# delta-mpc/delta-node

Measured on AMD Instinct MI355X. Metric: elements/s device-resident Shamir 3-of-5 split+recombine, 2^24 vec, 1/2/4/8 GPU, higher is better.
Workload: dtype u32

## Files before the change

delta-node_amd/csrc/dn_internal.hpp:

```cpp
#pragma once

#include <cstddef>
#include <cstdint>
#include <cstdlib>

#include "dn_shamir.h"

struct ihipEvent_t;
struct ihipStream_t;

namespace dn {
inline const char* tune_env(const char* name) {
#ifdef DN_TUNING
  return std::getenv(name);
#else
  (void)name;
  return nullptr;
#endif
}

int set_error(int code, const char* fmt, ...) __attribute__((format(printf, 2, 3)));

inline bool fd_needs_fold(int t, int n) {
  double s = 0.0, p = 1.0;
  for (int j = 0; j < t; ++j) {
    s += p;
    p *= static_cast<double>(n + t);
  }
  return s >= 8388608.0;
}

int device_cu_count();

struct StageBuf {
  void* p = nullptr;
  size_t bytes = 0;
  ::ihipEvent_t* ev = nullptr;
  int dev = -1;
};
StageBuf stage_take(size_t need);
void stage_give(StageBuf b, ::ihipStream_t* const* s);

uint64_t mt_jump_words();
uint64_t mt_jump_max_subs();
void mt_advance_window(const uint32_t* win, uint64_t steps, uint32_t* out);
bool mt_final_state(const uint32_t* state, int idx, uint64_t words, uint32_t* fin, int32_t* fidx);

constexpr uint64_t kMtRtRows = 2048;
const uint64_t* mt_direct_rows_l14(uint64_t S, uint64_t* version);
bool mt_rt_rows_compute(uint64_t* out, uint64_t nrows);
bool mt_xpow_mod(uint64_t e, uint64_t* out);
void mt_rt_rows_checksum(const uint64_t* words, uint64_t n, uint64_t out[2]);
}
```

delta-node_amd/csrc/host_gf2poly.cpp:

```cpp
#include <immintrin.h>

#include <cstdint>
#include <cstring>
#include <mutex>
#include <vector>

#include "dn_internal.hpp"

namespace dn {
namespace {

#include "mt19937_charpoly.inc"
#include "mt19937_jump.inc"
#include "mt19937_jump_direct.inc"

constexpr int kW = kMtPolyWords;
constexpr int kDeg = 19937;
static_assert(kW * 64 > kDeg && (kW - 1) * 64 <= kDeg, "poly words");

const uint64_t kP[1][kW] = DN_MT_CHAR_POLY;
const uint64_t kJump14[kMtJumpRows][kW] = DN_MT_JUMP_POLYS;
const uint64_t kDirect14[kMtDirectRows][kW] = DN_MT_JUMP_DIRECT_L14;

__attribute__((target("pclmul,sse4.1"))) void clmul_poly(const uint64_t* a, int na, const uint64_t* b, int nb,
                                                          uint64_t* r) {
  std::memset(r, 0, sizeof(uint64_t) * (na + nb));
  for (int k = 0; k < na + nb - 1; ++k) {
    const int i0 = k - nb + 1 > 0 ? k - nb + 1 : 0, i1 = k < na - 1 ? k : na - 1;
    __m128i acc = _mm_setzero_si128(), acc2 = _mm_setzero_si128();
    int i = i0;
    for (; i + 1 <= i1; i += 2) {
      const __m128i av = _mm_loadu_si128(reinterpret_cast<const __m128i*>(a + i));
      const __m128i bv = _mm_loadu_si128(reinterpret_cast<const __m128i*>(b + k - i - 1));
      acc = _mm_xor_si128(acc, _mm_clmulepi64_si128(av, bv, 0x10));
      acc2 = _mm_xor_si128(acc2, _mm_clmulepi64_si128(av, bv, 0x01));
    }
    if (i <= i1)
      acc = _mm_xor_si128(acc, _mm_clmulepi64_si128(_mm_loadl_epi64(reinterpret_cast<const __m128i*>(a + i)),
                                                     _mm_loadl_epi64(reinterpret_cast<const __m128i*>(b + k - i)), 0x00));
    acc = _mm_xor_si128(acc, acc2);
    r[k] ^= static_cast<uint64_t>(_mm_cvtsi128_si64(acc));
    r[k + 1] ^= static_cast<uint64_t>(_mm_extract_epi64(acc, 1));
  }
}

void shr_bits(const uint64_t* a, int na, int sh, uint64_t* out, int n) {
  const int ws = sh / 64, bs = sh % 64;
  for (int i = 0; i < n; ++i) {
    const int k = i + ws;
    const uint64_t lo = k < na ? a[k] : 0u;
    const uint64_t hi = k + 1 < na ? a[k + 1] : 0u;
    out[i] = bs ? (lo >> bs) | (hi << (64 - bs)) : lo;
  }
}

bool bit(const uint64_t* a, int i) { return (a[i / 64] >> (i % 64)) & 1u; }

// ... 64 lines not shown
    uint64_t h[2];
    mt_rt_rows_checksum(b, nw, h);
    if (h[0] != b[nw] || h[1] != b[nw + 1]) return nullptr;
    for (int s = 1; s <= kMtDirectRows; ++s)
      if (std::memcmp(b + (s - 1) * kW, kDirect14[s - 1], sizeof(uint64_t) * kW)) return nullptr;
    Barrett br;
    std::vector<uint64_t> r(kW);
    for (uint64_t s = kMtRtRows; s > kMtRtRows - 16 * 127; s -= 127) {
      br.mulmod(b + (s - 2) * kW, kJump14[kMtRowB + 1], r.data());
      if (std::memcmp(r.data(), b + (s - 1) * kW, sizeof(uint64_t) * kW)) return nullptr;
    }
    return b;
  }();
  return checked;
}

}

void mt_rt_rows_checksum(const uint64_t* w, uint64_t n, uint64_t out[2]) {
  uint64_t a = 0x9E3779B97F4A7C15ull ^ n, c = 0xC2B2AE3D27D4EB4Full;
  for (uint64_t i = 0; i < n; ++i) {
    a = ((a ^ w[i]) * 0xFF51AFD7ED558CCDull);
    a ^= a >> 29;
    c = ((c + w[i]) * 0xC4CEB9FE1A85EC53ull) ^ (c >> 31) ^ i;
  }
  out[0] = a;
  out[1] = c;
}

bool mt_xpow_mod(uint64_t e, uint64_t* out) {
  if (!__builtin_cpu_supports("pclmul")) return false;
  static Barrett* br = new Barrett;
  std::vector<uint64_t> r(kW, 0), t(kW);
  r[0] = 1;
  for (int b = e ? 63 - __builtin_clzll(e) : -1; b >= 0; --b) {
    br->mulmod(r.data(), r.data(), t.data());
    r.swap(t);
    if ((e >> b) & 1u) {
      uint64_t carry = 0;
      for (int k = 0; k < kW; ++k) {
        const uint64_t w = r[k];
        r[k] = (w << 1) | carry;
        carry = w >> 63;
      }
      if (bit(r.data(), kDeg)) {
        for (int k = 0; k < kW; ++k) r[k] ^= kP[0][k];
      }
    }
  }
  std::memcpy(out, r.data(), sizeof(uint64_t) * kW);
  return true;
}

bool mt_rt_rows_compute(uint64_t* out, uint64_t nrows) {
  if (!__builtin_cpu_supports("pclmul") || nrows == 0) return false;
  Barrett br;
  std::memcpy(out, kDirect14[0], sizeof(uint64_t) * kW);
  for (uint64_t s = 2; s <= nrows; ++s) {
    br.mulmod(out + (s - 2) * kW, kJump14[kMtRowB + 1], out + (s - 1) * kW);
    if (s <= static_cast<uint64_t>(kMtDirectRows) &&
        std::memcmp(out + (s - 1) * kW, kDirect14[s - 1], sizeof(uint64_t) * kW))
      return false;
  }
  return true;
}

const uint64_t* mt_direct_rows_l14(uint64_t S, uint64_t* version) {
  if (S < 2 || S - 1 > kMtRtRows) return nullptr;
  if (const uint64_t* e = embedded_rows()) {
    if (version) *version = ~0ull;
    return e;
  }
  if (!__builtin_cpu_supports("pclmul")) return nullptr;
  Rows& R = rows14();
  std::lock_guard<std::mutex> g(R.m);
  if (!R.ok) return nullptr;
  if (R.rows.empty()) {
    R.rows.assign(static_cast<size_t>(kMtRtRows) * kW, 0u);
    R.have.assign(kMtRtRows, 0u);
    R.br = new Barrett;
    std::memcpy(R.rows.data(), kDirect14[0], sizeof(uint64_t) * kW);
    R.have[0] = 1;
    R.odd_top = 1;
    if (!set_row(R, 2, R.rows.data(), kJump14[kMtRowB + 1])) return nullptr;
  }
  const uint64_t last = S - 1;
  for (uint64_t s = R.odd_top + 2; s <= last; s += 2, R.odd_top += 2)
    if (!set_row(R, s, R.rows.data() + (s - 3) * kW, kJump14[kMtRowB + 2])) return nullptr;
  if (!R.have[last - 1] && !set_row(R, last, R.rows.data() + (last - 2) * kW, kJump14[kMtRowB + 1]))
    return nullptr;
  if (version) *version = R.version;
  return R.rows.data();
}

}

extern "C" int dn_mt19937_rt_rows_embedded(void) { return dn::embedded_rows() ? 1 : 0; }
```

delta-node_amd/csrc/host_mt_jump.cpp:

```cpp
#include <cstdint>
#include <cstring>
#include <vector>

#include "dn_internal.hpp"

namespace dn {
namespace {

#include "mt19937_jump.inc"

alignas(64) static const uint64_t kMtJumpPolys[kMtJumpRows][kMtPolyWords] = DN_MT_JUMP_POLYS;

constexpr int kMtN = 624, kMtM = 397;
constexpr uint32_t kMtA = 0x9908b0dfu, kMtUp = 0x80000000u, kMtLo = 0x7fffffffu;

inline uint32_t mt_mix(uint32_t a, uint32_t b, uint32_t m) {
  const uint32_t y = (a & kMtUp) | (b & kMtLo);
  return m ^ (y >> 1) ^ ((0u - (y & 1u)) & kMtA);
}

__attribute__((target_clones("avx512f", "avx2", "default")))
void mt_extend(uint32_t* __restrict buf, uint64_t p, int steps) {
  const uint32_t* src = buf + p;
  uint32_t* dst = buf + p + kMtN;
// ... 70 lines not shown

uint64_t mt_jump_words() { return kMtJumpL; }
uint64_t mt_jump_max_subs() { return 1ull + static_cast<uint64_t>(kMtJumpRadix) * kMtJumpRadix * kMtJumpRadix; }

bool mt_final_state(const uint32_t* state, int idx, uint64_t words, uint32_t* fin, int32_t* fidx) {
  const uint64_t h = static_cast<uint64_t>(kMtN - idx);
  if (words <= h) {
    std::memcpy(fin, state, kMtN * sizeof(uint32_t));
    *fidx = idx + static_cast<int32_t>(words);
    return true;
  }
  const uint64_t m_end = words - h, q = (m_end + kMtN - 1) / kMtN, tf = kMtN * q;
  const uint64_t sig = (tf + kMtN - 1 - static_cast<uint64_t>(idx)) / kMtJumpL;
  if (sig >= mt_jump_max_subs()) return false;
  std::vector<uint32_t> w(kMtN);
  uint64_t t_sig = 0;
  if (sig == 0) {
    std::memcpy(w.data(), state, kMtN * sizeof(uint32_t));
  } else {
    mt_window_at(state, idx, sig, w.data());
    t_sig = static_cast<uint64_t>(idx) + sig * kMtJumpL - kMtN;
  }
  mt_advance(w.data(), tf - t_sig, fin);
  *fidx = static_cast<int32_t>(m_end - kMtN * (q - 1));
  return true;
}

void mt_advance_window(const uint32_t* win, uint64_t steps, uint32_t* out) { mt_advance(win, steps, out); }

}

using namespace dn;

extern "C" int dn_mt19937_skip(uint32_t* mt_state, int32_t* mt_index, uint64_t words) {
  if (!mt_state || !mt_index) return set_error(DN_ERR_ARG, "dn_mt19937_skip: null pointer");
  const int32_t idx = *mt_index;
  if (idx < 0 || idx > kMtN) return set_error(DN_ERR_ARG, "dn_mt19937_skip: bad MT index");
  std::vector<uint32_t> fin(kMtN);
  int32_t fidx = 0;
  if (!mt_final_state(mt_state, idx, words, fin.data(), &fidx))
    return set_error(DN_ERR_UNSUPPORTED, "dn_mt19937_skip: %llu words exceed the jump table",
                     static_cast<unsigned long long>(words));
  std::memcpy(mt_state, fin.data(), kMtN * sizeof(uint32_t));
  *mt_index = fidx;
  return DN_OK;
}

extern "C" int dn_mt19937_jump_poly(uint64_t words, uint64_t* out) {
  if (!out) return dn::set_error(DN_ERR_ARG, "dn_mt19937_jump_poly: null pointer");
  if (!dn::mt_xpow_mod(words, out))
    return dn::set_error(DN_ERR_UNSUPPORTED, "dn_mt19937_jump_poly: no carry-less multiply");
  return DN_OK;
}
```

delta-node_amd/csrc/mt19937_device.hip:

```cpp
#include <hip/hip_runtime.h>

#include <algorithm>
#include <cstdint>
#include <cstdlib>
#include <cstring>
#include <mutex>
#include <utility>
#include <vector>

#include "dn_internal.hpp"
#include "m521_device.hpp"
#include "mt_plan.hpp"
#include "seg_plan.hpp"

namespace dn {
namespace {

__device__ const uint64_t kMtPolysDev[kMtTabLens][kMtJumpRows][kMtPolyWords] = {
    DN_MT_JUMP_POLYS_L10, DN_MT_JUMP_POLYS_L12, DN_MT_JUMP_POLYS};
__device__ const uint64_t kMtDirectDev[kMtLens][kMtDirectRows][kMtPolyWords] = {
    DN_MT_JUMP_DIRECT_L10, DN_MT_JUMP_DIRECT_L12, DN_MT_JUMP_DIRECT_L14, DN_MT_JUMP_DIRECT_L8};

typedef uint32_t u32x2_t __attribute__((ext_vector_type(2)));
typedef uint32_t u32x4_t __attribute__((ext_vector_type(4)));
// ... 1198 lines not shown
}

struct MtKnobs {
  bool spec = true;
  bool tail_fin = true;
  bool spec_beside = true;
  int beside_cb = 2;
  uint64_t spec_min = 1ull << 23, beside_min = 1ull << 16;
  bool own_by_jumpc = false;
  uint32_t jump_probe = 0;
  bool jump4b = false;
  uint32_t gen_probe = 0;
  bool pc = true;
  uint32_t gen_subs = 0;
  bool force_retry = false;
};

MtKnobs mt_knobs() {
  MtKnobs k;
  auto on = [](const char* n, bool dflt) { const char* e = tune_env(n); return e ? e[0] != '0' : dflt; };
  auto is1 = [](const char* n) { const char* e = tune_env(n); return e && e[0] == '1'; };
  auto num = [](const char* n) { const char* e = tune_env(n); return e ? std::atoi(e) : 0; };
  k.spec = on("DN_MT_SPEC", k.spec);
  k.tail_fin = on("DN_MT_TAIL_FIN", k.tail_fin);
  k.spec_beside = on("DN_MT_SPEC_BESIDE", k.spec_beside);
  if (const char* e = tune_env("DN_MT_BESIDE_CB")) k.beside_cb = e[0] == '2' ? 2 : 3;
  if (const char* e = tune_env("DN_MT_SPEC_MIN")) k.spec_min = std::strtoull(e, nullptr, 10);
  if (const char* e = tune_env("DN_MT_BESIDE_MIN")) k.beside_min = std::strtoull(e, nullptr, 10);
  k.own_by_jumpc = num("DN_MT_SPEC_PROBE") == 5;
  k.jump_probe = static_cast<uint32_t>(num("DN_MT_JUMP_PROBE"));
  k.jump4b = is1("DN_MT_JUMP4B");
  k.gen_probe = static_cast<uint32_t>(num("DN_MT_PROBE"));
  k.pc = on("DN_MT_PC_FORCE", k.pc);
  if (tune_env("DN_MT_GEN_SUBS")) k.gen_subs = static_cast<uint32_t>(std::max(1, num("DN_MT_GEN_SUBS")));
  k.force_retry = is1("DN_MT_FORCE_RETRY");
  return k;
}

struct SpecState {
  std::mutex m;
  hipStream_t side = nullptr, side2 = nullptr;
  hipEvent_t win = nullptr, done = nullptr;
  hipEvent_t j0ev = nullptr, done2 = nullptr;
  bool widx2 = false;
  void* buf[2] = {nullptr, nullptr};
  uint64_t bytes = 0;
  bool armed = false;
  int next = 0;
  uint64_t ncoef = 0;
  int32_t idx = -1;
  uint32_t state[kMtN];
  bool have_end = false;
  uint64_t hits = 0, misses = 0, launched = 0;
  uint64_t* xpow = nullptr;
  uint64_t xpow_words = 0;
  bool xpow_failed = false;
};

std::mutex& spec_table_mutex() {
  static std::mutex* m = new std::mutex;
  return *m;
}
SpecState* spec_slot(int dev) {
  static SpecState* table[16] = {};
  if (dev < 0 || dev >= 16) return nullptr;
  std::lock_guard<std::mutex> g(spec_table_mutex());
  if (!table[dev]) {
    auto* x = new SpecState;
    if (hipStreamCreateWithFlags(&x->side, hipStreamNonBlocking) != hipSuccess ||
        hipStreamCreateWithFlags(&x->side2, hipStreamNonBlocking) != hipSuccess ||
        hipEventCreateWithFlags(&x->j0ev, hipEventDisableTiming) != hipSuccess ||
        hipEventCreateWithFlags(&x->done2, hipEventDisableTiming) != hipSuccess ||
        hipEventCreateWithFlags(&x->win, hipEventDisableTiming) != hipSuccess ||
        hipEventCreateWithFlags(&x->done, hipEventDisableTiming) != hipSuccess)
      return nullptr;
    table[dev] = x;
  }
  return table[dev];
}

bool spec_xpow(SpecState& sp, uint64_t words) {
  if (sp.xpow_failed) return false;
  if (sp.xpow && sp.xpow_words == words) return true;
  std::vector<uint64_t> g(kMtPolyWords);
  if (!mt_xpow_mod(words, g.data()) ||
      (!sp.xpow && hipMalloc(reinterpret_cast<void**>(&sp.xpow), kMtPolyWords * sizeof(uint64_t)) != hipSuccess)) {
    sp.xpow_failed = true;
    return false;
  }
  (void)hipStreamSynchronize(sp.side);
  (void)hipStreamSynchronize(sp.side2);
  if (hipMemcpy(sp.xpow, g.data(), kMtPolyWords * sizeof(uint64_t), hipMemcpyHostToDevice) != hipSuccess) {
    sp.xpow_failed = true;
    return false;
  }
  sp.xpow_words = words;
  return true;
}

bool spec_buffers(SpecState& sp, uint64_t need) {
  if (sp.bytes >= need && sp.buf[0] && sp.buf[1]) return true;
  (void)hipStreamSynchronize(sp.side);
  (void)hipStreamSynchronize(sp.side2);
  sp.armed = false;
  sp.widx2 = false;
  for (void*& b : sp.buf)
    if (b) (void)hipFree(b), b = nullptr;
  sp.bytes = 0;
  for (void*& b : sp.buf)
    if (hipMalloc(&b, need) != hipSuccess) {
      for (void*& c : sp.buf)
        if (c) (void)hipFree(c), c = nullptr;
      return false;
    }
  sp.bytes = need;
  return true;
}

constexpr uint64_t kCus = 256, kLdsPerCu = 160 * 1024;

struct SpecPlan {
  bool hit = false;
  bool spec_next = false;
  bool beside = false;
  bool widx2 = false;
  int dst = 0;
};

SpecPlan spec_decide(SpecState* sp, const MtKnobs& k, const MtHost& H, uint64_t ncoef, int ring_units, int32_t idx,
                     const uint32_t* mt_state) {
  SpecPlan p;
  if (!sp) return p;
  const bool cont = sp->have_end && sp->ncoef == ncoef && sp->idx == idx && !std::memcmp(sp->state, mt_state, kMtN * 4);
  p.hit = cont && sp->armed;
  if (sp->armed && !p.hit) ++sp->misses;
  p.widx2 = p.hit && sp->widx2;
  sp->armed = false;
  sp->widx2 = false;
  sp->have_end = false;
  p.spec_next = cont && spec_buffers(*sp, mt_scratch_bytes(ncoef));
  const uint64_t gen_lds = (1u + 2u * 17u * 64u * static_cast<uint32_t>(ring_units) + 64u) * 4u;
  const bool levels_fit = (H.S + kCus - 1) / kCus * gen_lds + (kEWords + kMtN + 64) * 4u <= kLdsPerCu;
  p.beside = p.spec_next && k.spec_beside && ncoef >= k.beside_min &&
             (H.rt ? !H.beside.jobs.empty() : levels_fit && (mt_sub_draws(H.ki) >= 4096 || H.S <= 256)) &&
             !H.j0.jobs.empty() && spec_xpow(*sp, 17 * ncoef);
  if (!p.beside && ncoef < k.spec_min) p.spec_next = false;
  p.dst = sp->next ^ 1;
  return p;
}

void spec_record_end(SpecState& sp, const SpecPlan& p, uint64_t ncoef, int32_t fidx, const uint32_t* mt_state) {
  sp.have_end = true;
  sp.ncoef = ncoef;
  sp.idx = fidx;
  std::memcpy(sp.state, mt_state, kMtN * 4);
  sp.armed = p.spec_next;
  sp.widx2 = p.beside;
  if (p.spec_next) sp.next = p.dst;
}

struct MtCall {
  const MtKnobs& k;
  const MtHost& H;
  hipStream_t s;
  uint8_t* sc;
  uint32_t* dwin;
  const void* jobs_dev;
  const uint64_t* rt_dev;
  SpecState* sp;
  SideStream* side;
};

hipError_t launch_levels(const MtCall& c, hipStream_t ls, uint32_t* wins, hipEvent_t after0 = nullptr) {
  const Level* lv = c.H.lv;
  const JumpJob* djobs = static_cast<const JumpJob*>(c.jobs_dev);
  const CombineJob* dcomb =
      reinterpret_cast<const CombineJob*>(djobs + lv[0].jobs.size() + lv[1].jobs.size() + lv[2].jobs.size());
  hipError_t err = hipSuccess;
  uint64_t off = 0, coff = 0;
  for (int k = 0; k < 3; ++k) {
    const Level& l = lv[k];
    if (!l.jobs.empty()) {
      const JumpArgs ja{wins, djobs + off, static_cast<uint32_t>(l.jobs.size()), c.k.jump_probe, c.rt_dev};
      const dim3 grid(static_cast<uint32_t>(l.jobs.size() / static_cast<size_t>(l.W)));
      if (l.W == 16 && c.k.jump4b) hipLaunchKernelGGL((mt_jumpc_kernel<16, 4>), grid, dim3(64 * 16), 0, ls, ja);
      else if (l.W == 16) hipLaunchKernelGGL(mt_jump_kernel<16>, grid, dim3(64 * 16), 0, ls, ja);
      else hipLaunchKernelGGL(mt_jump_kernel<8>, grid, dim3(64 * 8), 0, ls, ja);
    }
    if (!l.comb.empty())
      hipLaunchKernelGGL(mt_combine_kernel, dim3(static_cast<uint32_t>(l.comb.size())), dim3(640), 0, ls, wins,
                         dcomb + coff);
    off += l.jobs.size();
    coff += l.comb.size();
    if (after0 && k == 0) err = hipEventRecord(after0, ls);
  }
  return err;
}

void launch_beside_level(const MtCall& c, hipStream_t ls, uint32_t* wins) {
// ... 103 lines not shown
  ga.probe = c.k.gen_probe;
  if (tail_fin) ga.tail_fin = 1u, ga.fin_lo = fin.fin_lo, ga.next_lo = fin.next_lo;
  ga.sub_n = ga.S + (tail_fin ? 0u : 1u);
  return ga;
}

SpecState* spec_try_hold(std::unique_lock<std::mutex>& hold) {
  int dev = 0;
  SpecState* sp = hipGetDevice(&dev) == hipSuccess ? spec_slot(dev) : nullptr;
  if (sp) hold = std::unique_lock<std::mutex>(sp->m, std::try_to_lock);
  return sp && hold.owns_lock() ? sp : nullptr;
}

template <typename F>
int mt_device_run(const char* name, uint32_t* mt_state, int32_t* mt_index, uint64_t n_elem, int tm1, void* scratch,
                  uint64_t scratch_bytes, void* stream, int ring_units, F launch_gen) {
  if (!mt_state || !mt_index) return set_error(DN_ERR_ARG, "%s: null pointer", name);
  if (tm1 < 0 || tm1 >= DN_MAX_THRESHOLD) return set_error(DN_ERR_ARG, "%s: t-1=%d", name, tm1);
  const int32_t idx = *mt_index;
  if (idx < 0 || idx > kMtN) return set_error(DN_ERR_ARG, "%s: bad MT index", name);
  const uint64_t ncoef = n_elem * static_cast<uint64_t>(tm1);
  if (ncoef == 0) return DN_OK;
  if (!scratch) return set_error(DN_ERR_ARG, "%s: null pointer", name);
  const uint64_t S = mt_subs(ncoef);
  if (S > mt_jump_max_subs() - 1)
    return set_error(DN_ERR_UNSUPPORTED, "%s: %llu words exceed the jump table", name,
                     static_cast<unsigned long long>(17 * ncoef));
  if (scratch_bytes < mt_scratch_bytes(ncoef)) return set_error(DN_ERR_ARG, "%s: scratch too small", name);

  const MtKnobs k = mt_knobs();
  const int ki = mt_sub_len(ncoef);
  const MtFinal fin = mt_final_plan(idx, ncoef, S, ki);
  const bool tail_fin = fin.sig >= 0 && k.tail_fin;
  MtHost& H = mt_levels(S, ki);
  int jerr = 0;
  const void* jobs_dev = device_jobs(H, &jerr);
  if (jerr) return set_error(DN_ERR_HIP, "%s: job tables on the device", name);
  const uint64_t* rt_dev = H.rt ? device_rt(S, &jerr) : nullptr;
  if (jerr) return set_error(DN_ERR_HIP, "%s: runtime jump rows on the device", name);
  const size_t wpre = kHead / 4 + 2 * kMtN, wh = 256 / 4 + kMtN;
  PinLease lease(wpre + wh);
  uint32_t* pin = lease.p;
  if (!pin) return set_error(DN_ERR_HIP, "%s: pinned staging buffer", name);
  uint32_t *stw = pin + kHead / 4, *head = pin + wpre;
  std::memset(pin, 0, 256);
  mt_advance_window(mt_state, static_cast<uint64_t>(idx), stw);
  std::memcpy(stw + kMtN, mt_state, kMtN * 4);
  hipStream_t s = static_cast<hipStream_t>(stream);

  const bool spec_on = k.spec && !k.own_by_jumpc && !H.split2 && tail_fin && S >= 2 &&
                       ncoef >= std::min(k.spec_min, k.beside_min);
  std::unique_lock<std::mutex> spl;
  SpecState* sp = spec_on ? spec_try_hold(spl) : nullptr;
  const SpecPlan p = spec_decide(sp, k, H, ncoef, ring_units, idx, mt_state);
  uint8_t* sc = p.hit || p.beside ? static_cast<uint8_t*>(sp->buf[sp->next]) : static_cast<uint8_t*>(scratch);
  hipError_t err = (p.spec_next || p.hit) && hipEventQuery(sp->done) != hipSuccess ? hipStreamWaitEvent(s, sp->done, 0)
                                                                                   : hipSuccess;
  if (err == hipSuccess && (p.spec_next || p.hit) && hipEventQuery(sp->done2) != hipSuccess)
    err = hipStreamWaitEvent(s, sp->done2, 0);
  if (err == hipSuccess) err = hipMemcpyAsync(sc, pin, wpre * 4, hipMemcpyHostToDevice, s);
  if (err != hipSuccess) {
    (void)hipStreamSynchronize(s);
    return set_error(DN_ERR_HIP, "%s: %s", name, hipGetErrorString(err));
  }
  SideStream* side = H.split2 ? side_stream() : nullptr;
  if (H.split2 && !side) {
    (void)hipStreamSynchronize(s);
    return set_error(DN_ERR_HIP, "%s: side stream", name);
  }
  const MtCall c{k, H, s, sc, reinterpret_cast<uint32_t*>(sc + kHead) + kMtN, jobs_dev, rt_dev, sp, side};
  if (k.own_by_jumpc) launch_beside_level(c, s, c.dwin);
  else if (!p.hit) err = launch_levels(c, s, c.dwin, H.split2 ? side->levels : nullptr);

  head[0] = 0u;
  void* dhead = nullptr;
  if (hipHostGetDevicePointer(&dhead, head, 0) != hipSuccess || !dhead) {
    (void)hipStreamSynchronize(s);
    return set_error(DN_ERR_HIP, "%s: staging buffer not mapped", name);
  }
  GenArgs ga = gen_args(c, fin, tail_fin, idx, n_elem, tm1, static_cast<uint32_t*>(dhead));
  auto gen = [&](GenArgs& g, hipStream_t gs) { launch_gen(g, gs, k); };
  const MtLaunched r = H.split2      ? run_split2(c, ga, gen, err)
                       : p.beside    ? run_beside(c, p, ga, gen)
                       : p.spec_next ? run_spec_after(c, p, ga, gen)
                                     : run_plain(c, ga, gen, err);
  err = r.err;
  auto drain_side = [&]() {
    if (r.side_used) (void)hipStreamSynchronize(sp->side), (void)hipStreamSynchronize(sp->side2);
  };
  if (err != hipSuccess) {
    (void)hipStreamSynchronize(s);
    drain_side();
    return set_error(DN_ERR_HIP, "%s: side stream: %s", name, hipGetErrorString(err));
  }
  err = hipGetLastError();
  if (err != hipSuccess) {
    (void)hipStreamSynchronize(s);
    drain_side();
    return set_error(DN_ERR_HIP, "%s: launch: %s", name, hipGetErrorString(err));
  }
  err = hipStreamSynchronize(s);
  if (err != hipSuccess) {
    drain_side();
    return set_error(DN_ERR_HIP, "%s: %s", name, hipGetErrorString(err));
  }
  if (p.hit) ++sp->hits;
  if (head[0] || k.force_retry) return set_error(DN_ERR_RETRY, "%s: a draw was rejected; redo on the host", name);
  if (fin.sig >= 0) std::memcpy(mt_state, head + 256 / 4, kMtN * 4);
  *mt_index = fin.fidx;
  if (sp) spec_record_end(*sp, p, ncoef, fin.fidx, mt_state);
  return DN_OK;
}

constexpr int kSc1 = 16;

template <int T, bool SEG = false>
void launch_gen(GenArgs& ga, hipStream_t s, const MtKnobs& k) {
  ga.ring = 2u * 17u * 64u * (T ? T - 1 : 1);
  const uint32_t lds_words = 1u + ga.ring + 64u;
  uint32_t grid = ga.sub_n ? ga.sub_n : ga.S + 1;
  if (k.pc) {
    if (k.gen_subs) grid = std::min(grid, k.gen_subs);
    if (T == 3 && ga.n_shares == 5)
      hipLaunchKernelGGL((mt_gen_pc_kernel<T, kSc1, T == 3 ? 5 : 0, SEG>), dim3(grid), dim3(128), lds_words * 4u, s, ga);
    else
// ... 143 lines not shown
```

delta-node_amd/delta_node/crypto/shamir/_native.py:

```python
from __future__ import annotations

import array
import contextlib
import ctypes
import os
import threading
from typing import List, Optional, Sequence

import numpy as np

from . import _args

DN_OK = 0
DN_ERR_ARG = -1
DN_ERR_THRESHOLD = -2
DN_ERR_TOO_FEW = -3
DN_ERR_DISTINCT = -4
DN_ERR_HIP = -5
DN_ERR_UNSUPPORTED = -6
DN_ERR_EMPTY = -7
DN_ERR_RETRY = -8
DN_ERR_ZERODIV = -9
DN_ERR_ASSERT = -10
DN_ERR_OVERFLOW = -11
# ... 13 lines not shown
        ("neg", ctypes.c_uint32),
        ("shift", ctypes.c_int32),
        ("has_inv", ctypes.c_int32),
        ("d", ctypes.c_uint32),
        ("a", (ctypes.c_uint32 * 17) * MAX_RESOLVE),
        ("inv", ctypes.c_uint32 * 17),
        ("d_inv32", ctypes.c_uint32),
        ("p_inv_d", ctypes.c_uint32),
        ("d_recip", ctypes.c_uint64),
        ("w", ctypes.c_uint32 * 17),
        ("reserved", ctypes.c_uint32),
    ]


class Segment(ctypes.Structure):

    _fields_ = [("n_elem", ctypes.c_uint64), ("shares", ctypes.c_void_p)]


vp, u64, i32, cp = ctypes.c_void_p, ctypes.c_uint64, ctypes.c_int, ctypes.c_char_p
pvp, pu64, pu32, pi32 = (ctypes.POINTER(c) for c in (vp, u64, ctypes.c_uint32, ctypes.c_int32))
_SYMBOLS = {
    "dn_m521_vec_bytes": (u64, [u64], True),
    "dn_m521_split_u64": (i32, [vp, vp, vp, u64, i32, i32, vp], True),
    "dn_m521_split_fe": (i32, [vp, vp, vp, u64, i32, i32, vp], True),
    "dn_m521_lagrange": (i32, [pu64, i32, i32, ctypes.POINTER(Lagrange)], True),
    "dn_m521_reconstruct": (i32, [pvp, ctypes.POINTER(Lagrange), vp, vp, vp, u64, vp], True),
    "dn_mt19937_draw_coeffs": (i32, [pu32, pi32, u64, i32, vp], True),
    "dn_last_error": (cp, [], True),
    "dn_version": (cp, [], True),
    "dn_m521_split_prng": (i32, [vp, vp, u64, i32, u64, vp, u64, i32, i32, vp], True),
    "dn_m521_prng_coeffs": (i32, [vp, u64, i32, u64, vp, u64, i32, vp], True),
    "dn_mt19937_device_scratch_bytes": (u64, [u64, i32], True),
    "dn_mt19937_draw_coeffs_device": (i32, [vp, vp, u64, i32, vp, vp, u64, vp], True),
    "dn_mt19937_skip": (i32, [pu32, pi32, u64], True),
    "dn_mt19937_split_device": (i32, [vp, vp, vp, vp, u64, i32, i32, vp, u64, vp], True),
    "dn_mt19937_split_supported": (i32, [u64, i32, i32], True),
    "dn_shamir_make_shares_host": (i32, [cp, u64, cp, ctypes.c_uint32, i32, cp, ctypes.c_uint32, u64, vp, u64, vp],
                                   True),
    "dn_shamir_resolve_shares_host": (i32, [cp, vp, i32, i32, cp, ctypes.c_uint32, vp, u64, pu64], True),
    "dn_shamir_eval_at_host": (i32, [cp, vp, cp, i32, cp, ctypes.c_uint32, i32, cp, ctypes.c_uint32, i32, vp, u64,
                                     pu64, ctypes.POINTER(ctypes.c_int)], True),
    "dn_block_granularity": (i32, [i32, pu64], True),
    "dn_block_alloc": (i32, [u64, u64, i32, pvp], True),
    "dn_block_free": (i32, [vp], True),
    "dn_block_probe_rows": (i32, [vp, ctypes.c_uint32, u64, vp], True),
    "dn_block_record": (i32, [vp, vp], True),
    "dn_block_ready": (i32, [vp, vp, ctypes.POINTER(ctypes.c_int)], True),
    "dn_block_acquire": (i32, [vp, vp, i32], True),
    "dn_block_retired_bytes": (i32, [pu64], True),
    "dn_mt19937_rt_rows_embedded": (i32, [], True),
    "dn_mt19937_spec_stats": (i32, [pu64], False),
    "dn_mt19937_jump_poly": (i32, [u64, pu64], False),
    "dn_mt19937_split_many_scratch_bytes": (u64, [u64, i32, u64], False),
    "dn_mt19937_split_many_supported": (i32, [u64, i32, i32, u64], False),
    "dn_mt19937_split_many_device": (i32, [vp, vp, vp, ctypes.POINTER(Segment), u64, i32, i32, vp, u64, vp], False),
    "dn_m521_reconstruct_many_scratch_bytes": (u64, [u64, i32], False),
    "dn_m521_reconstruct_many": (i32, [pu64, pvp, pvp, pvp, vp, u64, ctypes.POINTER(Lagrange), vp, u64, vp], False),
    "dn_m521_sum_vecs": (i32, [pvp, cp, u64, vp, u64, vp], False),
    "dn_m521_reconstruct_records": (i32, [pvp, pu64, pvp, pu64, ctypes.POINTER(Lagrange), vp, vp, vp, vp, u64, vp],
                                    False),
    "dn_m521_sum_records": (i32, [pvp, pu64, pvp, u64, u64, cp, vp, vp, vp, u64, vp], False),
}
EXPORTS = tuple(_SYMBOLS)


def bind(L: ctypes.CDLL, table: dict, flag: str) -> ctypes.CDLL:
    if not getattr(L, flag, False):
        for name, (restype, argtypes, required) in table.items():
            if required or hasattr(L, name):
                fn = getattr(L, name)
                fn.restype, fn.argtypes = restype, argtypes
        setattr(L, flag, True)
    return L


def need(L: ctypes.CDLL, name: str) -> ctypes.CDLL:
    if not hasattr(L, name):
        raise RuntimeError(f"{lib_path()} lacks {name}: rebuild the native library")
    return L


_lock = threading.Lock()
_lib: Optional[ctypes.CDLL] = None


def lib_path() -> str:
    return os.environ.get("DN_SHAMIR_LIB", DEFAULT_LIB)


def lib() -> ctypes.CDLL:
    global _lib
    if _lib is not None:
        return _lib
    with _lock:
        if _lib is None:
            _lib = _load(lib_path())
        return _lib


@contextlib.contextmanager
def library(path: str):
    global _lib
    prev = lib()
    with _lock:
        _lib = _load(path)
# ... 349 lines not shown



def mt_split_device(rng, secrets, shares, n: int, t: int, n_shares: int) -> bool:
    import torch

    if n == 0:
        return True
    L = lib()
    shape = _mt_shape((id(L), n, t, n_shares), lambda: L.dn_mt19937_split_supported(n, t, n_shares),
                      lambda: L.dn_mt19937_device_scratch_bytes(n, t - 1))
    if not shape[0]:
        return False
    for name, x in (("secrets", secrets), ("shares", shares)):
        if not x.is_cuda or x.device != shares.device or not x.is_contiguous():
            raise ValueError(f"mt_split_device: {name} must be a contiguous tensor on the shares' HIP device")
    sb = shape[1]
    scratch = _mt_scratch(sb, shares.device)
    return _mt_device_draw(rng, lambda state, index: L.dn_mt19937_split_device(
        state, index, secrets.data_ptr(), shares.data_ptr(), n, t, n_shares, scratch.data_ptr(), sb, stream_ptr()))


def mt_split_many_device(rng, secrets, segs, t: int, n_shares: int) -> bool:
    n_total = sum(n for n, _ in segs)
    if n_total == 0:
        return True
    L = need(lib(), "dn_mt19937_split_many_device")
    shape = _mt_shape((id(L), n_total, t, n_shares, len(segs)),
                      lambda: L.dn_mt19937_split_many_supported(n_total, t, n_shares, len(segs)),
                      lambda: L.dn_mt19937_split_many_scratch_bytes(n_total, t - 1, len(segs)))
    if not shape[0]:
        return False
    dev = secrets.device
    if not secrets.is_cuda or not secrets.is_contiguous() or secrets.numel() != n_total:
        raise ValueError("mt_split_many_device: secrets must be a contiguous device tensor of the tensors' elements")
    table = (Segment * len(segs))(*segs)
    sb = shape[1]
    scratch = _mt_scratch(sb, dev)
    return _mt_device_draw(rng, lambda state, index: L.dn_mt19937_split_many_device(
        state, index, secrets.data_ptr(), table, len(segs), t, n_shares, scratch.data_ptr(), sb, stream_ptr()))


def mt_jump_poly(words: int):
    import numpy as np

    out = (ctypes.c_uint64 * 312)()
    check(lib().dn_mt19937_jump_poly(words, out))
    return np.frombuffer(out, dtype=np.uint64).copy()


def mt_spec_stats() -> dict:
    out = (ctypes.c_uint64 * 4)()
    check(lib().dn_mt19937_spec_stats(out))
    return {"hits": int(out[0]), "misses": int(out[1]), "launched": int(out[2]), "armed": bool(out[3])}


M521 = (1 << 521) - 1


def _prime_arg(prime: int):
    if prime == M521:
        return None, 0, 66
    pb = prime.to_bytes(max(1, (prime.bit_length() + 7) // 8), "big")
    return pb, len(pb), len(pb)


def host_make_shares(value: bytes, coeffs: Sequence[int], prime: int, threshold: int, n: int) -> List[bytes]:
    pb, plen, w = _prime_arg(prime)
    cb = b"".join([c.to_bytes(w, "big") for c in coeffs])
    cap = n * (9 + w)
    out = ctypes.create_string_buffer(cap)
    offs = (ctypes.c_uint64 * (n + 1))()
    rc = (_lib or lib()).dn_shamir_make_shares_host(value, len(value), cb, w, threshold, pb, plen, n, out, cap, offs)
    if rc:
        check(rc)
    raw = ctypes.string_at(out, offs[n])
    o = offs[:]
    return [raw[o[i]:o[i + 1]] for i in range(n)]


def host_resolve_shares(shares: Sequence[bytes], threshold: int, prime: int) -> bytes:
    pb, plen, w = _prime_arg(prime)
    k = len(shares)
    offs = (ctypes.c_uint64 * (k + 1))()
    o = 0
    for i, s in enumerate(shares):
        offs[i] = o
        o += len(s)
    offs[k] = o
    out = ctypes.create_string_buffer(w + 8)
    n = ctypes.c_uint64(0)
    rc = (_lib or lib()).dn_shamir_resolve_shares_host(b"".join(shares), offs, k, threshold, pb, plen, out, w + 8,
                                                       ctypes.byref(n))
    if rc:
        check(rc)
    return ctypes.string_at(out, n.value)


def _mag(v: int) -> bytes:
    v = abs(v)
    return v.to_bytes((v.bit_length() + 7) // 8, "big")


def host_eval_at(coeffs: Sequence[int], x: int, prime: int) -> int:
    k = len(coeffs)
    mags = [_mag(c) for c in coeffs]
    offs = (ctypes.c_uint64 * (k + 1))()
# ... 26 lines not shown
```

include/dn_shamir.h:

```cpp
#ifndef DN_SHAMIR_H
#define DN_SHAMIR_H

#include <stddef.h>
#include <stdint.h>

#ifdef __cplusplus
extern "C" {
#endif

#define DN_M521_LIMBS 17
#define DN_M521_TILE 256
#define DN_M521_TILE_BYTES 16896
#define DN_MAX_THRESHOLD 64
#define DN_MAX_SHARES 65535
#define DN_MAX_RESOLVE 16

enum {
  DN_OK = 0,
  DN_ERR_ARG = -1,
  DN_ERR_THRESHOLD = -2,
  DN_ERR_TOO_FEW = -3,
  DN_ERR_DISTINCT = -4,
  DN_ERR_HIP = -5,
  DN_ERR_UNSUPPORTED = -6,
// ... 53 lines not shown
                           int tm1, void* coeffs);

uint64_t dn_mt19937_device_scratch_bytes(uint64_t n_elem, int tm1);
int dn_mt19937_draw_coeffs_device(uint32_t* mt_state, int32_t* mt_index, uint64_t n_elem, int tm1,
                                  void* coeffs, void* scratch, uint64_t scratch_bytes, void* stream);

int dn_mt19937_split_device(uint32_t* mt_state, int32_t* mt_index, const int64_t* secrets, void* shares,
                            uint64_t n_elem, int threshold, int n_shares, void* scratch, uint64_t scratch_bytes,
                            void* stream);

int dn_mt19937_split_supported(uint64_t n_elem, int threshold, int n_shares);

typedef struct dn_m521_segment {
  uint64_t n_elem;
  void* shares;
} dn_m521_segment_t;

uint64_t dn_mt19937_split_many_scratch_bytes(uint64_t n_total, int tm1, uint64_t n_segments);
int dn_mt19937_split_many_supported(uint64_t n_total, int threshold, int n_shares, uint64_t n_segments);
int dn_mt19937_split_many_device(uint32_t* mt_state, int32_t* mt_index, const int64_t* secrets,
                                 const dn_m521_segment_t* segments, uint64_t n_segments, int threshold,
                                 int n_shares, void* scratch, uint64_t scratch_bytes, void* stream);

int dn_shamir_make_shares_host(const uint8_t* value, uint64_t value_len, const uint8_t* coeffs_be,
                               uint32_t coeff_bytes, int threshold, const uint8_t* prime_be, uint32_t prime_len,
                               uint64_t n_shares, uint8_t* out, uint64_t out_cap, uint64_t* offsets);
int dn_shamir_resolve_shares_host(const uint8_t* shares, const uint64_t* offsets, int k, int threshold,
                                  const uint8_t* prime_be, uint32_t prime_len, uint8_t* out, uint64_t out_cap,
                                  uint64_t* out_len);

int dn_shamir_eval_at_host(const uint8_t* coeffs_be, const uint64_t* coeff_offsets, const uint8_t* coeff_neg,
                           int n_coeffs, const uint8_t* x_be, uint32_t x_len, int x_neg, const uint8_t* prime_be,
                           uint32_t prime_len, int prime_neg, uint8_t* out, uint64_t out_cap, uint64_t* out_len,
                           int* out_neg);

int dn_block_granularity(int device, uint64_t* bytes);
int dn_block_alloc(uint64_t bytes, uint64_t chunk_bytes, int device, void** ptr);
int dn_block_free(void* ptr);
int dn_block_record(void* ptr, void* stream);
int dn_block_ready(void* ptr, void* stream, int* ready);
int dn_block_acquire(void* ptr, void* stream, int wait);
int dn_block_retired_bytes(uint64_t* bytes);

int dn_block_probe_rows(void* ptr, uint32_t rows, uint64_t row_bytes, void* stream);

int dn_mt19937_skip(uint32_t* mt_state, int32_t* mt_index, uint64_t words);

int dn_mt19937_rt_rows_embedded(void);

int dn_mt19937_spec_stats(uint64_t* out);

int dn_mt19937_jump_poly(uint64_t words, uint64_t* out);

uint64_t dn_m521_codec_scratch_bytes(uint64_t n_elem);
uint64_t dn_m521_encoded_capacity(uint64_t n_elem, uint64_t x);
int dn_m521_encode_shares(const void* vec, uint64_t n_elem, uint64_t x, uint64_t* offsets, uint8_t* out,
                          uint64_t capacity, void* scratch, uint64_t scratch_bytes, void* stream);
int dn_m521_decode_shares(const uint8_t* in, uint64_t in_bytes, const uint64_t* offsets, uint64_t n_elem, void* vec,
                          uint64_t* xs, uint32_t* bad_count, void* stream);

uint64_t dn_m521_encode_many_scratch_bytes(uint64_t n_segments, uint64_t total_tiles, uint64_t n_rows);
int dn_m521_encode_shares_many(const uint64_t* n_elem, const void* const* blocks, const uint64_t* pitches,
                               uint64_t n_segments, const uint32_t* rows, const uint64_t* xs,
                               uint64_t* const* offsets, uint8_t* const* outs, const uint64_t* capacities,
                               uint64_t n_rows, uint64_t* totals, void* scratch, uint64_t scratch_bytes,
                               void* stream);

int dn_m521_reconstruct_records(const uint8_t* const* in, const uint64_t* in_bytes,
                                const uint64_t* const* offsets, const uint64_t* xs,
                                const dn_m521_lagrange_t* w, void* out_fe, int64_t* out_u64,
                                uint32_t* overflow_count, uint32_t* bad_counts ,
                                uint64_t n_elem, void* stream);

#define DN_M521_SUM_RECORDS_GROUP 64
int dn_m521_sum_records(const uint8_t* const* in, const uint64_t* in_bytes, const uint64_t* const* offsets,
                        uint64_t m, uint64_t x, const uint8_t* negate, const void* acc, void* out,
                        uint32_t* bad_counts , uint64_t n_elem, void* stream);

#define DN_M521_FRAME_GROUP 64
uint64_t dn_m521_frame_records_offset(uint64_t n_elem);
uint64_t dn_m521_frame_capacity(uint64_t n_elem, uint64_t x);
int dn_m521_frame_finish(const uint64_t* const* offsets, uint8_t* const* frames, const uint64_t* xs, uint64_t m,
                         uint64_t n_elem, void* stream);
uint64_t dn_m521_frame_scratch_bytes(uint64_t n_elem, uint64_t m);
int dn_m521_frame_open(const uint8_t* const* frames, const uint64_t* frame_bytes, const uint64_t* xs, uint64_t m,
                       uint64_t n_elem, uint64_t* const* offsets_out, uint32_t* bad_counts ,
                       void* scratch, uint64_t scratch_bytes, void* stream);

const char* dn_last_error(void);

const char* dn_version(void);

#ifdef __cplusplus
}
#endif

#endif
```

Measured before the change: 11.44 billion.

## Compute MT jump polynomials asynchronously on a worker thread with slot cache

Replaces the synchronous host computation of the x^e mod P jump polynomial, along with its blocking stream syncs and hipMemcpy, with a multi-slot cache filled by a detached background thread. Device copies are staged through pinned memory with hipMemcpyAsync and ordered across the side streams using an event. Speculative buffer growth is deferred until after the main launches. Calls that find the polynomial not yet ready fall back to the non-beside path, which removes host stalls on the critical path. In exchange it adds a thread, locking and more complex state, and the beside path may be skipped early on.

```diff
diff --git a/delta-node_amd/csrc/dn_internal.hpp b/delta-node_amd/csrc/dn_internal.hpp
--- a/delta-node_amd/csrc/dn_internal.hpp
+++ b/delta-node_amd/csrc/dn_internal.hpp
@@ -50,5 +50,8 @@
 const uint64_t* mt_direct_rows_l14(uint64_t S, uint64_t* version);
 bool mt_rt_rows_compute(uint64_t* out, uint64_t nrows);
 bool mt_xpow_mod(uint64_t e, uint64_t* out);
+constexpr int kMtXpowSlots = 8;
+int mt_xpow_cached(uint64_t e, uint64_t* out, int* slot, uint64_t* gen);
+void mt_xpow_cache_stats(uint64_t out[2]);
 void mt_rt_rows_checksum(const uint64_t* words, uint64_t n, uint64_t out[2]);
 }
diff --git a/delta-node_amd/csrc/host_gf2poly.cpp b/delta-node_amd/csrc/host_gf2poly.cpp
--- a/delta-node_amd/csrc/host_gf2poly.cpp
+++ b/delta-node_amd/csrc/host_gf2poly.cpp
@@ -1,8 +1,14 @@
 #include <immintrin.h>
 
+#include <pthread.h>
+#include <signal.h>
+
+#include <condition_variable>
 #include <cstdint>
 #include <cstring>
 #include <mutex>
+#include <system_error>
+#include <thread>
 #include <vector>
 
 #include "dn_internal.hpp"
@@ -173,6 +179,102 @@
   return true;
 }
 
+namespace {
+struct XpowCache {
+  enum State { kEmpty, kQueued, kReady, kFailed };
+  struct Ent {
+    uint64_t e = 0, gen = 0, used = 0;
+    State state = kEmpty;
+    uint64_t poly[kW];
+  };
+  std::mutex m;
+  std::condition_variable cv;
+  Ent ent[kMtXpowSlots];
+  uint64_t tick = 0, gens = 0, queued = 0, evicted = 0;
+  bool worker = false;
+};
+
+XpowCache& xpow_cache() {
+  static XpowCache* c = new XpowCache;
+  return *c;
+}
+
+void xpow_worker() {
+  XpowCache& c = xpow_cache();
+  std::vector<uint64_t> r(kW);
+  std::unique_lock<std::mutex> lk(c.m);
+  for (;;) {
+    XpowCache::Ent* job = nullptr;
+    for (XpowCache::Ent& x : c.ent)
+      if (x.state == XpowCache::kQueued && (!job || x.gen < job->gen)) job = &x;
+    if (!job) {
+      c.cv.wait(lk);
+      continue;
+    }
+    const uint64_t e = job->e;
+    lk.unlock();
+    const bool ok = mt_xpow_mod(e, r.data());
+    lk.lock();
+    std::memcpy(job->poly, r.data(), sizeof(uint64_t) * kW);
+    job->state = ok ? XpowCache::kReady : XpowCache::kFailed;
+  }
+}
+
+bool start_xpow_worker() {
+  sigset_t all, old;
+  sigfillset(&all);
+  const bool masked = pthread_sigmask(SIG_SETMASK, &all, &old) == 0;
+  bool ok = true;
+  try {
+    std::thread(xpow_worker).detach();
+  } catch (const std::system_error&) {
+    ok = false;
+  }
+  if (masked) (void)pthread_sigmask(SIG_SETMASK, &old, nullptr);
+  return ok;
+}
+}
+
+int mt_xpow_cached(uint64_t e, uint64_t* out, int* slot, uint64_t* gen) {
+  if (!__builtin_cpu_supports("pclmul")) return -1;
+  XpowCache& c = xpow_cache();
+  std::lock_guard<std::mutex> g(c.m);
+  for (int i = 0; i < kMtXpowSlots; ++i) {
+    XpowCache::Ent& x = c.ent[i];
+    if (x.state == XpowCache::kEmpty || x.e != e) continue;
+    x.used = ++c.tick;
+    if (x.state != XpowCache::kReady) return x.state == XpowCache::kFailed ? -1 : 0;
+    if (out) std::memcpy(out, x.poly, sizeof(uint64_t) * kW);
+    if (slot) *slot = i;
+    if (gen) *gen = x.gen;
+    return 1;
+  }
+  int v = -1;
+  for (int i = 0; i < kMtXpowSlots && (v < 0 || c.ent[v].state != XpowCache::kEmpty); ++i) {
+    const XpowCache::Ent& x = c.ent[i];
+    if (x.state == XpowCache::kQueued) continue;
+    if (v < 0 || x.state == XpowCache::kEmpty || x.used < c.ent[v].used) v = i;
+  }
+  if (v < 0) return 0;
+  if (!c.worker && !(c.worker = start_xpow_worker())) return -1;
+  XpowCache::Ent& x = c.ent[v];
+  if (x.state != XpowCache::kEmpty) ++c.evicted;
+  x.e = e;
+  x.gen = ++c.gens;
+  x.used = ++c.tick;
+  x.state = XpowCache::kQueued;
+  ++c.queued;
+  c.cv.notify_one();
+  return 0;
+}
+
+void mt_xpow_cache_stats(uint64_t out[2]) {
+  XpowCache& c = xpow_cache();
+  std::lock_guard<std::mutex> g(c.m);
+  out[0] = c.queued;
+  out[1] = c.evicted;
+}
+
 bool mt_rt_rows_compute(uint64_t* out, uint64_t nrows) {
   if (!__builtin_cpu_supports("pclmul") || nrows == 0) return false;
   Barrett br;
diff --git a/delta-node_amd/csrc/host_mt_jump.cpp b/delta-node_amd/csrc/host_mt_jump.cpp
--- a/delta-node_amd/csrc/host_mt_jump.cpp
+++ b/delta-node_amd/csrc/host_mt_jump.cpp
@@ -146,3 +146,18 @@
     return dn::set_error(DN_ERR_UNSUPPORTED, "dn_mt19937_jump_poly: no carry-less multiply");
   return DN_OK;
 }
+
+extern "C" int dn_mt19937_jump_poly_cached(uint64_t words, uint64_t* out, int* ready) {
+  if (!out || !ready) return dn::set_error(DN_ERR_ARG, "dn_mt19937_jump_poly_cached: null pointer");
+  const int r = dn::mt_xpow_cached(words, out, nullptr, nullptr);
+  if (r < 0)
+    return dn::set_error(DN_ERR_UNSUPPORTED, "dn_mt19937_jump_poly_cached: no carry-less multiply, or no thread");
+  *ready = r;
+  return DN_OK;
+}
+
+extern "C" int dn_mt19937_jump_poly_stats(uint64_t* out) {
+  if (!out) return dn::set_error(DN_ERR_ARG, "dn_mt19937_jump_poly_stats: null pointer");
+  dn::mt_xpow_cache_stats(out);
+  return DN_OK;
+}
diff --git a/delta-node_amd/csrc/mt19937_device.hip b/delta-node_amd/csrc/mt19937_device.hip
--- a/delta-node_amd/csrc/mt19937_device.hip
+++ b/delta-node_amd/csrc/mt19937_device.hip
@@ -1274,8 +1274,9 @@
   uint32_t state[kMtN];
   bool have_end = false;
   uint64_t hits = 0, misses = 0, launched = 0;
-  uint64_t* xpow = nullptr;
-  uint64_t xpow_words = 0;
+  uint64_t *xpow_dev = nullptr, *xpow_pin = nullptr;
+  uint64_t xpow_gen[kMtXpowSlots] = {};
+  const uint64_t* xpow = nullptr;
   bool xpow_failed = false;
 };
 
@@ -1296,32 +1297,46 @@
         hipEventCreateWithFlags(&x->win, hipEventDisableTiming) != hipSuccess ||
         hipEventCreateWithFlags(&x->done, hipEventDisableTiming) != hipSuccess)
       return nullptr;
+    const size_t pb = kMtXpowSlots * kMtPolyWords * sizeof(uint64_t);
+    void *d = nullptr, *h = nullptr;
+    if (hipMalloc(&d, pb) != hipSuccess || hipHostMalloc(&h, pb, hipHostMallocDefault) != hipSuccess) {
+      if (d) (void)hipFree(d);
+      x->xpow_failed = true;
+    } else {
+      x->xpow_dev = static_cast<uint64_t*>(d);
+      x->xpow_pin = static_cast<uint64_t*>(h);
+    }
     table[dev] = x;
   }
   return table[dev];
 }
 
-bool spec_xpow(SpecState& sp, uint64_t words) {
-  if (sp.xpow_failed) return false;
-  if (sp.xpow && sp.xpow_words == words) return true;
-  std::vector<uint64_t> g(kMtPolyWords);
-  if (!mt_xpow_mod(words, g.data()) ||
-      (!sp.xpow && hipMalloc(reinterpret_cast<void**>(&sp.xpow), kMtPolyWords * sizeof(uint64_t)) != hipSuccess)) {
-    sp.xpow_failed = true;
-    return false;
-  }
-  (void)hipStreamSynchronize(sp.side);
-  (void)hipStreamSynchronize(sp.side2);
-  if (hipMemcpy(sp.xpow, g.data(), kMtPolyWords * sizeof(uint64_t), hipMemcpyHostToDevice) != hipSuccess) {
-    sp.xpow_failed = true;
-    return false;
-  }
-  sp.xpow_words = words;
-  return true;
-}
+int spec_xpow(SpecState& sp, uint64_t words) {
+  if (sp.xpow_failed) return -1;
+  uint64_t g[kMtPolyWords], gen = 0;
+  int slot = 0;
+  const int r = mt_xpow_cached(words, g, &slot, &gen);
+  if (r < 0) sp.xpow_failed = true;
+  if (r <= 0) return r;
+  uint64_t* d = sp.xpow_dev + static_cast<size_t>(slot) * kMtPolyWords;
+  if (sp.xpow_gen[slot] != gen) {
+    if (hipEventQuery(sp.done) != hipSuccess || hipEventQuery(sp.done2) != hipSuccess) return 0;
+    uint64_t* pin = sp.xpow_pin + static_cast<size_t>(slot) * kMtPolyWords;
+    std::memcpy(pin, g, sizeof(g));
+    sp.xpow_gen[slot] = 0;
+    if (hipMemcpyAsync(d, pin, sizeof(g), hipMemcpyHostToDevice, sp.side) != hipSuccess ||
+        hipEventRecord(sp.j0ev, sp.side) != hipSuccess || hipStreamWaitEvent(sp.side2, sp.j0ev, 0) != hipSuccess)
+      return 0;
+    sp.xpow_gen[slot] = gen;
+  }
+  sp.xpow = d;
+  return 1;
+}
+
+bool spec_have_buffers(const SpecState& sp, uint64_t need) { return sp.bytes >= need && sp.buf[0] && sp.buf[1]; }
 
 bool spec_buffers(SpecState& sp, uint64_t need) {
-  if (sp.bytes >= need && sp.buf[0] && sp.buf[1]) return true;
+  if (spec_have_buffers(sp, need)) return true;
   (void)hipStreamSynchronize(sp.side);
   (void)hipStreamSynchronize(sp.side2);
   sp.armed = false;
@@ -1346,6 +1361,7 @@
   bool spec_next = false;
   bool beside = false;
   bool widx2 = false;
+  bool grow = false;
   int dst = 0;
 };
 
@@ -1360,13 +1376,17 @@
   sp->armed = false;
   sp->widx2 = false;
   sp->have_end = false;
-  p.spec_next = cont && spec_buffers(*sp, mt_scratch_bytes(ncoef));
+  p.spec_next = cont;
+  p.grow = cont && !spec_have_buffers(*sp, mt_scratch_bytes(ncoef));
   const uint64_t gen_lds = (1u + 2u * 17u * 64u * static_cast<uint32_t>(ring_units) + 64u) * 4u;
   const bool levels_fit = (H.S + kCus - 1) / kCus * gen_lds + (kEWords + kMtN + 64) * 4u <= kLdsPerCu;
-  p.beside = p.spec_next && k.spec_beside && ncoef >= k.beside_min &&
-             (H.rt ? !H.beside.jobs.empty() : levels_fit && (mt_sub_draws(H.ki) >= 4096 || H.S <= 256)) &&
-             !H.j0.jobs.empty() && spec_xpow(*sp, 17 * ncoef);
-  if (!p.beside && ncoef < k.spec_min) p.spec_next = false;
+  const bool beside_shape = k.spec_beside && ncoef >= k.beside_min &&
+                            (H.rt ? !H.beside.jobs.empty() : levels_fit && (mt_sub_draws(H.ki) >= 4096 || H.S <= 256)) &&
+                            !H.j0.jobs.empty();
+  const int xp = p.spec_next && beside_shape ? spec_xpow(*sp, 17 * ncoef) : -1;
+  p.beside = xp == 1 && !p.grow;
+  if (!p.beside && xp < 0 && ncoef < k.spec_min) p.spec_next = false;
+  p.grow = p.grow && p.spec_next;
   p.dst = sp->next ^ 1;
   return p;
 }
@@ -1576,7 +1596,7 @@
                        ncoef >= std::min(k.spec_min, k.beside_min);
   std::unique_lock<std::mutex> spl;
   SpecState* sp = spec_on ? spec_try_hold(spl) : nullptr;
-  const SpecPlan p = spec_decide(sp, k, H, ncoef, ring_units, idx, mt_state);
+  SpecPlan p = spec_decide(sp, k, H, ncoef, ring_units, idx, mt_state);
   uint8_t* sc = p.hit || p.beside ? static_cast<uint8_t*>(sp->buf[sp->next]) : static_cast<uint8_t*>(scratch);
   hipError_t err = (p.spec_next || p.hit) && hipEventQuery(sp->done) != hipSuccess ? hipStreamWaitEvent(s, sp->done, 0)
                                                                                    : hipSuccess;
@@ -1595,6 +1615,7 @@
   const MtCall c{k, H, s, sc, reinterpret_cast<uint32_t*>(sc + kHead) + kMtN, jobs_dev, rt_dev, sp, side};
   if (k.own_by_jumpc) launch_beside_level(c, s, c.dwin);
   else if (!p.hit) err = launch_levels(c, s, c.dwin, H.split2 ? side->levels : nullptr);
+  if (p.grow && !spec_buffers(*sp, mt_scratch_bytes(ncoef))) p.spec_next = false;
 
   head[0] = 0u;
   void* dhead = nullptr;
diff --git a/delta-node_amd/delta_node/crypto/shamir/_native.py b/delta-node_amd/delta_node/crypto/shamir/_native.py
--- a/delta-node_amd/delta_node/crypto/shamir/_native.py
+++ b/delta-node_amd/delta_node/crypto/shamir/_native.py
@@ -89,6 +89,8 @@
     "dn_mt19937_rt_rows_embedded": (i32, [], True),
     "dn_mt19937_spec_stats": (i32, [pu64], False),
     "dn_mt19937_jump_poly": (i32, [u64, pu64], False),
+    "dn_mt19937_jump_poly_cached": (i32, [u64, pu64, ctypes.POINTER(ctypes.c_int)], False),
+    "dn_mt19937_jump_poly_stats": (i32, [pu64], False),
     "dn_mt19937_split_many_scratch_bytes": (u64, [u64, i32, u64], False),
     "dn_mt19937_split_many_supported": (i32, [u64, i32, i32, u64], False),
     "dn_mt19937_split_many_device": (i32, [vp, vp, vp, ctypes.POINTER(Segment), u64, i32, i32, vp, u64, vp], False),
@@ -544,7 +546,21 @@
 def mt_spec_stats() -> dict:
     out = (ctypes.c_uint64 * 4)()
     check(lib().dn_mt19937_spec_stats(out))
-    return {"hits": int(out[0]), "misses": int(out[1]), "launched": int(out[2]), "armed": bool(out[3])}
+    res = {"hits": int(out[0]), "misses": int(out[1]), "launched": int(out[2]), "armed": bool(out[3])}
+    if hasattr(lib(), "dn_mt19937_jump_poly_stats"):
+        pc = (ctypes.c_uint64 * 2)()
+        check(lib().dn_mt19937_jump_poly_stats(pc))
+        res["polys"], res["polys_evicted"] = int(pc[0]), int(pc[1])
+    return res
+
+
+def mt_jump_poly_cached(words: int):
+    import numpy as np
+
+    out = (ctypes.c_uint64 * 312)()
+    ready = ctypes.c_int(0)
+    check(lib().dn_mt19937_jump_poly_cached(words, out, ctypes.byref(ready)))
+    return np.frombuffer(out, dtype=np.uint64).copy() if ready.value else None
 
 
 M521 = (1 << 521) - 1
diff --git a/include/dn_shamir.h b/include/dn_shamir.h
--- a/include/dn_shamir.h
+++ b/include/dn_shamir.h
@@ -129,6 +129,10 @@
 
 int dn_mt19937_jump_poly(uint64_t words, uint64_t* out);
 
+int dn_mt19937_jump_poly_cached(uint64_t words, uint64_t* out, int* ready);
+
+int dn_mt19937_jump_poly_stats(uint64_t* out);
+
 uint64_t dn_m521_codec_scratch_bytes(uint64_t n_elem);
 uint64_t dn_m521_encoded_capacity(uint64_t n_elem, uint64_t x);
 int dn_m521_encode_shares(const void* vec, uint64_t n_elem, uint64_t x, uint64_t* offsets, uint8_t* out,
```

After: 11.28 billion. -1.4%, worse.
